# physiii/radio-mapper

Measured on AMD Instinct MI355X. Metric: IQ samples cross-correlated per second, higher is better.
Workload: dtype f32; 1 GPU; cfg3: 8 buoys (28 pairs), 10 MS/s complex64, N=4096-sample windows (L=8192), 4096 windows per GPU resident in HBM; n_buoys=8, n_pairs=28, n_samples=4096, windows_per_gpu=4096, channels=1, windows_total=4096, parallelism=windows sharded x1, no collective

## Files before the change

__graft_entry__.py:

```python
import os
import subprocess
import sys

ROOT = os.path.dirname(os.path.abspath(__file__))
CSRC = os.path.join(ROOT, "radio-mapper_amd", "csrc")
HIPCC = os.environ.get("HIPCC", "/opt/rocm/bin/hipcc")
HIP_FLAGS = ["--offload-arch=gfx950", "-O3", "-std=c++17", "-fPIC", "-shared", "-fno-slp-vectorize",
             "-mllvm", "-simplifycfg-sink-common=false",
             "-Wno-inline-asm"]
SOURCES = ("rmx_hip.hip", "fft_r16.hpp", "fft_r8.hpp", "kwin.hpp", "kwin8k.hpp", "kwin16k.hpp", "generic_path.hpp", "win_eo.hpp", "host_plan.hpp",
           "detect_path.hpp", "lag_bounds.hpp", "kwin_body.hpp", "xspec_weight.hpp", "integrate.hpp")
LIB = os.path.join(CSRC, "librmx_hip.so")
_MARK = b"RMX_BUILD_INFO source_digest="


def source_digest() -> str:
    import hashlib
    h = hashlib.sha256()
    for f in sorted(os.listdir(CSRC)):
        if f.endswith((".hip", ".hpp")):
            h.update(f.encode())
            h.update(open(os.path.join(CSRC, f), "rb").read())
    h.update(open(os.path.join(ROOT, "include", "rmx.h"), "rb").read())
    h.update(" ".join(HIP_FLAGS).encode())
    return h.hexdigest()[:16]


def binary_digest(path: str = LIB):
    try:
        blob = open(path, "rb").read()
    except OSError:
        return None
    k = blob.find(_MARK)
    if k < 0:
        return None
    k += len(_MARK)
    return blob[k:k + 16].decode("ascii", "replace")


def _stale(target=LIB) -> bool:
    return binary_digest(target) != source_digest()


def build(force: bool = False) -> None:
    for f in SOURCES:
        assert os.path.exists(os.path.join(CSRC, f)), f
    lib = LIB
    if force or _stale(lib):
        cmd = [HIPCC] + HIP_FLAGS + [f'-DRMX_SOURCE_DIGEST="{source_digest()}"', "-o", lib, os.path.join(CSRC, "rmx_hip.hip")]
        print("[build]", " ".join(cmd), flush=True)
        subprocess.run(cmd, check=True)
    else:
        print("[build] up to date (binary digest == source digest %s): no compile" % source_digest(), flush=True)
    if ROOT not in sys.path:
        sys.path.insert(0, ROOT)
    import radio_mapper_amd
    from radio_mapper_amd import xcorr
    lib_h = xcorr.load_library()
    assert lib_h.rmx_version() >= 1
    info = xcorr.build_info()
    assert info.get("source_digest") == source_digest(), (info, source_digest())
    print("[build] ok:", lib, info["text"], "devices visible:", xcorr.device_count(), flush=True)


def smoke() -> None:
    if ROOT not in sys.path:
        sys.path.insert(0, ROOT)
    import numpy as np
    import radio_mapper_amd as rm
    from radio_mapper_amd import xcorr
    from oracle import xcorr_ref as orc
    iq, delays, raw = rm.synth.make_windows(8, 4, 4096, 10e6, seed=7, return_u8=True)
    ri, rf, rp = orc.xcorr_batch_literal(iq)
    ref = ri + rf
    worst = 0.0
    for fused in (0, 1):
        with xcorr.XcorrEngine(4, 4096, 8, device=0) as eng:
            if fused:
                eng.set_option("small4096", 0)
            li, lf, pk = eng.correlate(iq)
            li8, lf8, pk8 = eng.correlate(raw)
        assert np.array_equal(li, ri), "integer lags differ from the oracle"
        assert np.all(np.abs(li + lf.astype(np.float64) - ref) <= 1e-5 * np.maximum(np.abs(ref), 1.0))
        assert np.allclose(pk, rp, rtol=1e-5)
        assert np.array_equal(li, li8) and np.array_equal(lf, lf8)
        worst = max(worst, float(np.abs(li + lf - ref).max()))
    print("[smoke] ok: 8 windows x 6 pairs through both N = 4096 paths, lag_int bit-exact, max |dlag| = %.2e" % worst, flush=True)


if __name__ == "__main__":
    build()
    if len(sys.argv) > 1 and sys.argv[1] == "smoke":
        smoke()
```

radio-mapper_amd/csrc/fft_r16.hpp:

```cpp
#pragma once
#include <hip/hip_runtime.h>

#include <type_traits>

namespace rmx {

constexpr int kM = 4096;
constexpr int kL = 2 * kM;
constexpr int kThreads = 512;
constexpr int kSlots = 16;

__device__ __forceinline__ float2 cmul(float2 a, float2 b) {
    return make_float2(a.x * b.x - a.y * b.y, a.x * b.y + a.y * b.x);
}
__device__ __forceinline__ float2 cadd(float2 a, float2 b) { return make_float2(a.x + b.x, a.y + b.y); }
__device__ __forceinline__ float2 csub(float2 a, float2 b) { return make_float2(a.x - b.x, a.y - b.y); }

__device__ __forceinline__ void dft4(float2& a0, float2& a1, float2& a2, float2& a3) {
    const float2 t0 = cadd(a0, a2), t1 = csub(a0, a2);
    const float2 t2 = cadd(a1, a3), t3 = csub(a1, a3);
    a0 = cadd(t0, t2);
    a2 = csub(t0, t2);
    a1 = make_float2(t1.x + t3.y, t1.y - t3.x);
    a3 = make_float2(t1.x - t3.y, t1.y + t3.x);
// ... 48 lines not shown
    const float ax = a.x, ay = a.y;
    a.x = b.x; a.y = b.y;
    b.x = ax; b.y = ay;
}

__device__ __forceinline__ void dft16_layer2(float2 (&v)[16]) {
    dft4(v[0], v[1], v[2], v[3]);
    dft4_tw<true>(v[4], v[5], v[6], v[7], make_float2(1.f, 0.f), make_float2(RMX_C1, -RMX_S1),
                  make_float2(RMX_RH, -RMX_RH), make_float2(RMX_S1, -RMX_C1));
    {
        float2 &a0 = v[8], &a1 = v[9], &a2 = v[10], &a3 = v[11];
        const float2 t0 = make_float2(a0.x + a2.y, a0.y - a2.x);
        const float2 t1 = make_float2(a0.x - a2.y, a0.y + a2.x);
        const float2 A1 = make_float2((a1.x + a1.y) * RMX_RH, (a1.y - a1.x) * RMX_RH);
        const float2 t2 = cfma(A1, a3, make_float2(-RMX_RH, -RMX_RH));
        const float2 t3 = twice_minus(A1, t2);
        dft4_tail(a0, a1, a2, a3, t0, t1, t2, t3);
    }
    dft4_tw<true>(v[12], v[13], v[14], v[15], make_float2(1.f, 0.f), make_float2(RMX_S1, -RMX_C1),
                  make_float2(-RMX_RH, -RMX_RH), make_float2(-RMX_C1, RMX_S1));
    swap2(v[1], v[4]);
    swap2(v[2], v[8]);
    swap2(v[3], v[12]);
    swap2(v[6], v[9]);
    swap2(v[7], v[13]);
    swap2(v[11], v[14]);
}

template <class F>
__device__ __forceinline__ void dft16_layer2_emit(float2 (&v)[16], F&& emit) {
    dft4(v[0], v[1], v[2], v[3]);
    emit(std::integral_constant<int, 0>{}, v[0], v[1], v[2], v[3]);
    __builtin_amdgcn_sched_barrier(0);
    dft4_tw<true>(v[4], v[5], v[6], v[7], make_float2(1.f, 0.f), make_float2(RMX_C1, -RMX_S1),
                  make_float2(RMX_RH, -RMX_RH), make_float2(RMX_S1, -RMX_C1));
    emit(std::integral_constant<int, 1>{}, v[4], v[5], v[6], v[7]);
    __builtin_amdgcn_sched_barrier(0);
    {
        float2 &a0 = v[8], &a1 = v[9], &a2 = v[10], &a3 = v[11];
        const float2 t0 = make_float2(a0.x + a2.y, a0.y - a2.x);
        const float2 t1 = make_float2(a0.x - a2.y, a0.y + a2.x);
        const float2 A1 = make_float2((a1.x + a1.y) * RMX_RH, (a1.y - a1.x) * RMX_RH);
        const float2 t2 = cfma(A1, a3, make_float2(-RMX_RH, -RMX_RH));
        const float2 t3 = twice_minus(A1, t2);
        dft4_tail(a0, a1, a2, a3, t0, t1, t2, t3);
    }
    emit(std::integral_constant<int, 2>{}, v[8], v[9], v[10], v[11]);
    __builtin_amdgcn_sched_barrier(0);
    dft4_tw<true>(v[12], v[13], v[14], v[15], make_float2(1.f, 0.f), make_float2(RMX_S1, -RMX_C1),
                  make_float2(-RMX_RH, -RMX_RH), make_float2(-RMX_C1, RMX_S1));
    emit(std::integral_constant<int, 3>{}, v[12], v[13], v[14], v[15]);
    __builtin_amdgcn_sched_barrier(0);
}

__device__ __forceinline__ void dft16(float2 (&v)[16]) {
    dft4(v[0], v[4], v[8], v[12]);
    dft4(v[1], v[5], v[9], v[13]);
    dft4(v[2], v[6], v[10], v[14]);
    dft4(v[3], v[7], v[11], v[15]);
    dft16_layer2(v);
}

template <bool W0_IS_ONE>
__device__ __forceinline__ void dft16_tw(float2 (&v)[16], const float2 (&w)[16]) {
    dft4_tw<W0_IS_ONE>(v[0], v[4], v[8], v[12], w[0], w[4], w[8], w[12]);
    dft4_tw<false>(v[1], v[5], v[9], v[13], w[1], w[5], w[9], w[13]);
    dft4_tw<false>(v[2], v[6], v[10], v[14], w[2], w[6], w[10], w[14]);
    dft4_tw<false>(v[3], v[7], v[11], v[15], w[3], w[7], w[11], w[15]);
    dft16_layer2(v);
}

struct C16 {
    float re[16], im[16];
    __device__ __forceinline__ float2 get(int q) const { return make_float2(re[q], im[q]); }
    __device__ __forceinline__ void set(int q, float x, float y) { re[q] = x; im[q] = y; }
};
template <bool W0_IS_ONE>
__device__ __forceinline__ void dft16_tw_l1(float2 (&v)[16], const C16& w) {
    dft4_tw<W0_IS_ONE>(v[0], v[4], v[8], v[12], w.get(0), w.get(4), w.get(8), w.get(12));
    dft4_tw<false>(v[1], v[5], v[9], v[13], w.get(1), w.get(5), w.get(9), w.get(13));
    dft4_tw<false>(v[2], v[6], v[10], v[14], w.get(2), w.get(6), w.get(10), w.get(14));
    dft4_tw<false>(v[3], v[7], v[11], v[15], w.get(3), w.get(7), w.get(11), w.get(15));
}
template <bool W0_IS_ONE>
__device__ __forceinline__ void dft16_tw(float2 (&v)[16], const C16& w) {
    dft16_tw_l1<W0_IS_ONE>(v, w);
    dft16_layer2(v);
}

__device__ __forceinline__ void dft16_tw_row_l1(float2 (&v)[16], const float4* row, float4 f0, float4 f1) {
    dft4_tw<true>(v[0], v[4], v[8], v[12], make_float2(1.0f, 0.0f), make_float2(f0.x, f0.y), make_float2(f0.z, f0.w),
                  make_float2(f1.x, f1.y));
    const float4 f2 = row[2], f3 = row[3];
    dft4_tw<false>(v[1], v[5], v[9], v[13], make_float2(f1.z, f1.w), make_float2(f2.x, f2.y), make_float2(f2.z, f2.w),
                   make_float2(f3.x, f3.y));
    const float4 f4 = row[4], f5 = row[5];
    dft4_tw<false>(v[2], v[6], v[10], v[14], make_float2(f3.z, f3.w), make_float2(f4.x, f4.y), make_float2(f4.z, f4.w),
                   make_float2(f5.x, f5.y));
    const float4 f6 = row[6], f7 = row[7];
    dft4_tw<false>(v[3], v[7], v[11], v[15], make_float2(f5.z, f5.w), make_float2(f6.x, f6.y), make_float2(f6.z, f6.w),
                   make_float2(f7.x, f7.y));
}
__device__ __forceinline__ void dft16_tw_row_l1(float2 (&v)[16], const float4* row) {
    dft16_tw_row_l1(v, row, row[0], row[1]);
}
__device__ __forceinline__ void dft16_tw_row(float2 (&v)[16], const float4* row, float4 f0, float4 f1) {
    dft16_tw_row_l1(v, row, f0, f1);
    dft16_layer2(v);
}
__device__ __forceinline__ void dft16_tw_row(float2 (&v)[16], const float4* row) {
    dft16_tw_row_l1(v, row);
    dft16_layer2(v);
}

__device__ __forceinline__ void cmul_inplace(float& x, float& y, float wr, float wi) {
    float tmp;
    asm volatile("v_mul_f32 %2, %0, %4\n\tv_mul_f32 %0, %0, %3\n\tv_fma_f32 %0, -%1, %4, %0\n\tv_fma_f32 %1, %1, %3, %2"
                 : "+v"(x), "+v"(y), "=&v"(tmp)
                 : "s"(wr), "s"(wi));
}

__device__ __forceinline__ void cmul4_inplace(float& x0, float& y0, float& x1, float& y1, float& x2, float& y2,
                                              float& x3, float& y3, float2 w0, float2 w1, float2 w2, float2 w3) {
    float tmp;
#define RMX_CM(X, Y, WR, WI)                                                                              \
    "v_mul_f32 %8, %" #X ", %" #WI "\n\tv_mul_f32 %" #X ", %" #X ", %" #WR "\n\tv_fma_f32 %" #X ", -%" #Y \
    ", %" #WI ", %" #X "\n\tv_fma_f32 %" #Y ", %" #Y ", %" #WR ", %8\n\t"
    asm volatile(RMX_CM(0, 1, 9, 10) RMX_CM(2, 3, 11, 12) RMX_CM(4, 5, 13, 14) RMX_CM(6, 7, 15, 16)
                 : "+v"(x0), "+v"(y0), "+v"(x1), "+v"(y1), "+v"(x2), "+v"(y2), "+v"(x3), "+v"(y3), "=&v"(tmp)
                 : "s"(w0.x), "s"(w0.y), "s"(w1.x), "s"(w1.y), "s"(w2.x), "s"(w2.y), "s"(w3.x), "s"(w3.y));
#undef RMX_CM
}

__device__ __forceinline__ float2 w32(int q) {
    constexpr float c[16] = {1.0f, 0.98078528040323044913f, 0.92387953251128675613f,
                             0.83146961230254523708f, 0.70710678118654752440f,
                             0.55557023301960222474f, 0.38268343236508977173f,
                             0.19509032201612826785f, 0.0f, -0.19509032201612826785f,
                             -0.38268343236508977173f, -0.55557023301960222474f,
                             -0.70710678118654752440f, -0.83146961230254523708f,
                             -0.92387953251128675613f, -0.98078528040323044913f};
    constexpr float s[16] = {0.0f, 0.19509032201612826785f, 0.38268343236508977173f,
                             0.55557023301960222474f, 0.70710678118654752440f,
                             0.83146961230254523708f, 0.92387953251128675613f,
                             0.98078528040323044913f, 1.0f, 0.98078528040323044913f,
                             0.92387953251128675613f, 0.83146961230254523708f,
                             0.70710678118654752440f, 0.55557023301960222474f,
                             0.38268343236508977173f, 0.19509032201612826785f};
    return make_float2(c[q], -s[q]);
}

constexpr int kBcRow = 34;
constexpr int kBcHalf = 16 * kBcRow;
constexpr int kXchgF2 = 16 * kBcHalf;

__device__ __forceinline__ void wave_lds_fence() {
    __builtin_amdgcn_fence(__ATOMIC_RELEASE, "wavefront");
    __builtin_amdgcn_s_waitcnt(0xC07F);
    __builtin_amdgcn_wave_barrier();
    __builtin_amdgcn_fence(__ATOMIC_ACQUIRE, "wavefront");
}

__device__ __forceinline__ void wave_lds_order() {
    __builtin_amdgcn_fence(__ATOMIC_RELEASE, "wavefront");
    __builtin_amdgcn_wave_barrier();
    __builtin_amdgcn_fence(__ATOMIC_ACQUIRE, "wavefront");
// ... 184 lines not shown
```

radio-mapper_amd/csrc/kwin.hpp:

```cpp
#pragma once
#include <hip/hip_runtime.h>

#include <cmath>
#include <type_traits>
#include <vector>

#include "fft_r16.hpp"

#ifndef RMX_KWIN_LOAD_AUX
#define RMX_KWIN_LOAD_AUX 0
#endif
#ifndef RMX_KWIN_STORE_AUX
#define RMX_KWIN_STORE_AUX 0
#endif

namespace rmx {

using u32x4 = unsigned int __attribute__((ext_vector_type(4)));
using u32x2 = unsigned int __attribute__((ext_vector_type(2)));
using f32x4 = float __attribute__((ext_vector_type(4)));
using f32x2 = float __attribute__((ext_vector_type(2)));

constexpr int kLdsXchg = kXchgF2 * 8;
constexpr int kLdsTw2 = 16 * kTw2RowF2 * 8;
constexpr int kLdsRed = 64;
constexpr int kLdsBytes = kLdsXchg + kLdsTw2 + kLdsRed;

__device__ __forceinline__ void load_tw2_to_lds(float2* tw2_lds, const float2* __restrict__ tw2_g, int t) {
    if (t < 256) tw2_lds[(t >> 4) * kTw2RowF2 + (t & 15)] = tw2_g[t];
}

__device__ __forceinline__ void load_tw2_to_lds_grouped(float2* tw2_lds, const float2* __restrict__ tw2_g, int t) {
    if (t < 256) {
        const int a = t >> 4, q = t & 15;
        tw2_lds[a * kTw2RowF2 + (q == 0 ? 15 : 4 * (q & 3) + (q >> 2) - 1)] = tw2_g[t];
    }
}

__device__ __forceinline__ void load_tw1(float2 (&tw1)[16], const float4* __restrict__ tw1_g, int t) {
#pragma unroll
    for (int j = 0; j < 8; ++j) {
        const float4 w = tw1_g[j * kThreads + t];
        tw1[2 * j] = make_float2(w.x, w.y);
        tw1[2 * j + 1] = make_float2(w.z, w.w);
    }
}

constexpr int kLdsWinImg = kLdsXchg;
constexpr int kLdsWinTw2 = 2 * kLdsWinImg;
#ifdef RMX_KWIN_PEAK2
constexpr int kResSlots = 4;
constexpr int kResBatch = 3;
constexpr int kHaloRows = 7;
#ifndef RMX_KWIN_RES_MASK
#define RMX_KWIN_RES_MASK 3
#endif
#else
#ifndef RMX_KWIN_RES_MASK
#define RMX_KWIN_RES_MASK 7
#endif
constexpr int kResSlots = 8;
constexpr int kResBatch = 7;
constexpr int kHaloRows = 4;
#endif
constexpr int kLdsWinHalo = kLdsWinTw2 + kLdsTw2;
constexpr int kLdsWinRed = kLdsWinHalo + kResSlots * 8 * kHaloRows * 16 * 4;
constexpr int kLdsWinOidx = kLdsWinRed + kResSlots * 8 * 16;
constexpr int kLdsWinBytes = kLdsWinOidx + kResSlots * 4;
static_assert(kLdsWinBytes <= 160 * 1024, "k_win LDS");

__device__ __forceinline__ void k_to_owner(int kk, int& tt, int& q) {
    const int par = (kk >= kM - 1) ? 0 : 1;
    const int n = par ? (kk + 1) : (kk - (kM - 1));
    tt = 2 * (n & 255) + par;
    q = n >> 8;
}

template <bool BOUNDED = false>
__device__ __forceinline__ void resolve_batch(int lane, const float4* red, const float* halo, const int* oidx,
                                              int first, int cnt, long obase, float out_scale,
                                              int* __restrict__ lag_int, float* __restrict__ lag_frac,
                                              float* __restrict__ peak, LagBounds lb = {}, long w = 0) {
    const int g = lane >> 3, r = lane & 7;
    const bool act = g < cnt;
    const int slot = (first + g) & (kResSlots - 1);
    const float* rf = reinterpret_cast<const float*>(red) + 4 * (slot * 8 + r);
    const int* ri = reinterpret_cast<const int*>(rf);
    const float ex = act ? rf[0] : -3.0f;
    const int k = act ? ri[1] : 0x7fffffff;
    const float tm = rf[2], tp = rf[3];
    const int out = oidx[slot];
    float gmax = ex;
    gmax = fmaxf(gmax, __builtin_bit_cast(float, dpp_i<0xB1>(__builtin_bit_cast(int, gmax))));
    gmax = fmaxf(gmax, __builtin_bit_cast(float, dpp_i<0x4E>(__builtin_bit_cast(int, gmax))));
    gmax = fmaxf(gmax, __builtin_bit_cast(float, dpp_i<0x141>(__builtin_bit_cast(int, gmax))));
    int kstar = (ex == gmax) ? k : 0x7fffffff;
// ... 160 lines not shown
```

radio-mapper_amd/csrc/kwin_body.hpp:

```cpp
#ifdef RMX_ABLATE
    const int dbg = dbg_rt;
#else
    constexpr int dbg = 0;
    (void)dbg_rt;
#endif
    extern __shared__ __attribute__((aligned(16))) char smem[];
    float2* img0 = reinterpret_cast<float2*>(smem);
    float2* img1 = reinterpret_cast<float2*>(smem + kLdsWinImg);
    float2* tw2_lds = reinterpret_cast<float2*>(smem + kLdsWinTw2);
    float* halo = reinterpret_cast<float*>(smem + kLdsWinHalo);
    float4* red = reinterpret_cast<float4*>(smem + kLdsWinRed);
    int* oidx = reinterpret_cast<int*>(smem + kLdsWinOidx);

    const int t = threadIdx.x;
    const int p = t & 1, u = t >> 1;
    const int lane = t & 63, wave = t >> 6;
    const int B = n_buoys;
    const int n_pairs = B * (B - 1) / 2;

    load_tw2_to_lds_grouped(tw2_lds, tw2_g, t);
    float2 tw1[16];
    load_tw1(tw1, tw1_g, t);
#ifndef RMX_KWIN_LDS1
    const float4* tw2row = reinterpret_cast<const float4*>(tw2_lds + (t & 15) * kTw2RowF2);
// ... 73 lines not shown
                resolve_batch(lane, red, halo, oidx, (npair - npend) & (kResSlots - 1), npend, obase, out_scale, lag_int,
                              lag_frac, peak);
            }
#endif
            npend = 0;
        }
    };
    auto mul_w32_odd = [&](float2 (&v)[16]) __attribute__((always_inline)) {
        if (p) {
            {
#pragma unroll
                for (int q = 1; q < 4; ++q) {
                    const float2 w = w32(q);
                    float x = v[q].x, y = v[q].y;
                    cmul_inplace(x, y, w.x, w.y);
                    v[q].x = x;
                    v[q].y = y;
                }
            }
#pragma unroll
            for (int q = 4; q < 16; q += 4) {
                float x0 = v[q].x, y0 = v[q].y, x1 = v[q + 1].x, y1 = v[q + 1].y;
                float x2 = v[q + 2].x, y2 = v[q + 2].y, x3 = v[q + 3].x, y3 = v[q + 3].y;
                cmul4_inplace(x0, y0, x1, y1, x2, y2, x3, y3, w32(q), w32(q + 1), w32(q + 2), w32(q + 3));
                v[q].x = x0; v[q].y = y0; v[q + 1].x = x1; v[q + 1].y = y1;
                v[q + 2].x = x2; v[q + 2].y = y2; v[q + 3].x = x3; v[q + 3].y = y3;
            }
        }
    };
    const int samp_bytes = U8 ? 2 : 8;
    const __amdgpu_buffer_rsrc_t xs = __builtin_amdgcn_make_buffer_rsrc(
        const_cast<char*>(reinterpret_cast<const char*>(iq_v)) + (first_window + wl) * (long)B * kM * samp_bytes, 0,
        B * kM * samp_bytes, 0x00020000);
    const __amdgpu_buffer_rsrc_t ss = __builtin_amdgcn_make_buffer_rsrc(
        reinterpret_cast<char*>(spec) + wbase * (long)(8 * kThreads * 16), 0, B * (8 * kThreads * 16), 0x00020000);
    const int xoff = u * samp_bytes, soff = t * 16;
    auto load_x = [&](C16& d, int b) __attribute__((always_inline)) {
        if constexpr (U8) {
#pragma unroll
            for (int q = 0; q < 16; ++q)
                d.re[q] = __uint_as_float((unsigned)__builtin_amdgcn_raw_buffer_load_b16(xs, xoff, (b * kM + q * 256) * 2, 0));
        } else {
#pragma unroll
            for (int q = 0; q < 16; ++q) {
                const u32x2 r = __builtin_amdgcn_raw_buffer_load_b64(xs, xoff, (b * kM + q * 256) * 8, 0);
                d.set(q, __uint_as_float(r.x), __uint_as_float(r.y));
            }
        }
    };
    auto load_x_part_from = [&](const __amdgpu_buffer_rsrc_t& rs, C16& d, int b, auto part) __attribute__((always_inline)) {
        constexpr int G = decltype(part)::value;
        if (dbg & 64) return;
#ifndef RMX_KWIN_NO_SPREAD
        constexpr int Q0 = 2 * G, Q1 = 2 * G + 2;
#else
        constexpr int Q0 = 4 * G, Q1 = 4 * G + 4;
#endif
        int bo = b * (kM * samp_bytes);
        asm volatile("" : "+s"(bo));
        if constexpr (U8) {
#pragma unroll
            for (int q = Q0; q < Q1; ++q)
                d.re[q] = __uint_as_float((unsigned)__builtin_amdgcn_raw_buffer_load_b16(rs, xoff, bo + q * 256 * 2, 0));
        } else {
#pragma unroll
            for (int q = Q0; q < Q1; ++q) {
                const u32x2 r = __builtin_amdgcn_raw_buffer_load_b64(rs, xoff, bo + q * 256 * 8, 0);
                d.set(q, __uint_as_float(r.x), __uint_as_float(r.y));
            }
        }
    };
    auto load_x_part = [&](C16& d, int b, auto part) __attribute__((always_inline)) { load_x_part_from(xs, d, b, part); };
    auto cvt_x = [&](C16& d) __attribute__((always_inline)) {
        if constexpr (U8) {
#pragma unroll
            for (int q = 0; q < 16; ++q) {
                const unsigned r = __float_as_uint(d.re[q]);
                d.set(q, (float)(r & 0xffu) - 127.5f, (float)(r >> 8) - 127.5f);
            }
        }
    };
    auto load_spec_part = [&](C16& d, int b, auto part) __attribute__((always_inline)) {
        constexpr int G = decltype(part)::value;
        if (dbg & 32) b = 1;
        if (dbg & 128) return;
#ifndef RMX_KWIN_NO_SPREAD
        constexpr int J0 = G, J1 = G + 1;
#else
        constexpr int J0 = 2 * G, J1 = 2 * G + 2;
#endif
        int bo = b * (8 * kThreads * 16);
        asm volatile("" : "+s"(bo));
#pragma unroll
        for (int j = J0; j < J1; ++j) {
            const u32x4 w = __builtin_amdgcn_raw_buffer_load_b128(ss, soff, bo + j * (kThreads * 16), RMX_KWIN_LOAD_AUX);
            d.set(2 * j, __uint_as_float(w.x), __uint_as_float(w.y));
            d.set(2 * j + 1, __uint_as_float(w.z), __uint_as_float(w.w));
        }
    };
    auto store_spec = [&](const C16& d, int b) __attribute__((always_inline)) {
#pragma unroll
        for (int j = 0; j < 8; ++j) {
            float e0 = d.re[2 * j], e1 = d.im[2 * j], e2 = d.re[2 * j + 1], e3 = d.im[2 * j + 1];
            asm volatile("" : "+v"(e0), "+v"(e1), "+v"(e2), "+v"(e3));
            const u32x4 w = {__float_as_uint(e0), __float_as_uint(e1), __float_as_uint(e2), __float_as_uint(e3)};
            __builtin_amdgcn_raw_buffer_store_b128(w, ss, soff + (b * 8 + j) * (kThreads * 16), 0, RMX_KWIN_STORE_AUX);
        }
    };
    auto fwd = [&](C16& xc) __attribute__((always_inline)) {
        float2* img = (seq & 1) ? img1 : img0;
        float2 x[16];
#ifdef RMX_KWIN_STAMPS
        RMX_LAP(6);
        asm volatile("s_waitcnt vmcnt(0)" ::: "memory");
        RMX_LAP(7);
#endif
#pragma unroll
        for (int q = 0; q < 16; ++q) x[q] = xc.get(q);
        mul_w32_odd(x);
        dft16(x);
        mul_tw1(x, tw1);
#ifndef RMX_KWIN_LDS1
        if (!(dbg & 8)) xchg_a2_write(img, x, t);
        RMX_LAP(0);
        barrier_hook(false);
        RMX_LAP(1);
        if (!(dbg & 8)) xchg_b2_read(img, x, t);
#else
        if (!(dbg & 8)) xchg_a_write(img, x, t);
        barrier_hook(false);
        if (!(dbg & 8)) xchg_b_read(img, x, t);
#endif
        dft16(x);
#ifdef RMX_TW2_LDS
        const float4 r0 = tw2row[0], r1 = tw2row[1];
#endif
        if (!(dbg & 4)) {
#ifndef RMX_KWIN_LDS1
        loc_write16(loc_m0[seq & 1], x);
        wave_lds_order();
        loc_read16(smem + (seq & 1) * kLdsWinImg + loc_rd, x);
#else
        xchg_bc_write_b(img, x, t);
        wave_lds_order();
        xchg_bc_read_c(img, x, t);
#endif
        }
#ifndef RMX_TW2_LDS
        dft16_tw<true>(x, tw2r);
#else
        dft16_tw_row(x, tw2row, r0, r1);
#endif
#pragma unroll
        for (int q = 0; q < 16; ++q) xc.set(q, x[q].x, x[q].y);
        ++seq;
        RMX_LAP(2);
    };
    auto pair_h1 = [&](const C16& a, const C16& s, int tr, auto prefetch) __attribute__((always_inline)) {
        float2* img = (tr & 1) ? img1 : img0;
        float2 v[16];
#ifdef RMX_KWIN_STAMPS
        {
            const long long c0 = __builtin_readcyclecounter();
            asm volatile("s_waitcnt vmcnt(0)" ::: "memory");
            const long long c1 = __builtin_readcyclecounter();
            stamp_vm += (int)(c1 - c0);
        }
#endif
#pragma unroll
        for (int q = 0; q < 16; ++q) v[q] = make_float2(s.im[q], s.re[q]);
        dft16_tw_l1<false>(v, a);
#pragma unroll
        for (int q = 0; q < 16; q += 4)
            asm volatile("" : "+v"(v[q].x), "+v"(v[q].y), "+v"(v[q + 1].x), "+v"(v[q + 1].y), "+v"(v[q + 2].x),
                         "+v"(v[q + 2].y), "+v"(v[q + 3].x), "+v"(v[q + 3].y));
        __builtin_amdgcn_sched_barrier(0);
        {
            float2* wb = img + (u >> 4) * kBcHalf + (u & 15) * kBcRow + p;
            (void)wb;
            dft16_layer2_emit(v, [&](auto kac, const float2& x0, const float2& x1, const float2& x2, const float2& x3)
                                     __attribute__((always_inline)) {
                constexpr int ka = decltype(kac)::value;
                if (!(dbg & 4)) {
#ifndef RMX_KWIN_LDS1
                    loc_write4<ka, ka + 4, ka + 8, ka + 12>(loc_m0[tr & 1], x0, x1, x2, x3);
#else
                    wb[2 * ka] = make_float2(x0.x, x0.y);
                    wb[2 * (ka + 4)] = make_float2(x1.x, x1.y);
                    wb[2 * (ka + 8)] = make_float2(x2.x, x2.y);
                    wb[2 * (ka + 12)] = make_float2(x3.x, x3.y);
#endif
                }
                if (!(dbg & 16)) prefetch(kac);
            });
        }
#ifdef RMX_TW2_LDS
        const float4 r0 = tw2row[0], r1 = tw2row[1];
#endif
        if (!(dbg & 4)) {
            wave_lds_order();
#ifndef RMX_KWIN_LDS1
            loc_read16(smem + (tr & 1) * kLdsWinImg + loc_rd, v);
#else
            xchg_bc_read_b(img, v, t);
#endif
        }
#ifndef RMX_TW2_LDS
        dft16_tw_l1<true>(v, tw2r);
#else
        dft16_tw_row_l1(v, tw2row, r0, r1);
#endif
        {
#ifndef RMX_KWIN_LDS1
            float2* xb = img + xb2_base(t);
#else
            float2* xb = img + (u >> 4) * kBcHalf + (u & 15) * 2 + p;
#endif
            dft16_layer2_emit(v, [&](auto kac, const float2& x0, const float2& x1, const float2& x2, const float2& x3)
                                     __attribute__((always_inline)) {
                constexpr int ka = decltype(kac)::value;
                if (!(dbg & 8)) {
                    xb[ka * 32] = make_float2(x0.x, x0.y);
                    xb[(ka + 4) * 32] = make_float2(x1.x, x1.y);
                    xb[(ka + 8) * 32] = make_float2(x2.x, x2.y);
                    xb[(ka + 12) * 32] = make_float2(x3.x, x3.y);
                }
#ifndef RMX_KWIN_NO_SPREAD
                if (!(dbg & 16)) prefetch(std::integral_constant<int, ka + 4>{});
#endif
            });
        }
    };
    auto pair_h2 = [&](int tr, int out_idx) __attribute__((always_inline)) {
        const float2* img = (tr & 1) ? img1 : img0;
        const int rb = npair & (kResSlots - 1);
        float2 v[16];
#ifndef RMX_KWIN_LDS1
        if (!(dbg & 8)) xchg_a2_read(img, v, t);
#else
        if (!(dbg & 8)) xchg_a_read(img, v, t);
#endif
        dft16_tw<false>(v, tw1);
        mul_w32_odd(v);
        pair_fmac8(v[0].x, v[0].y, v[1].x, v[1].y, v[2].x, v[2].y, v[3].x, v[3].y, sgn);
        pair_fmac8(v[4].x, v[4].y, v[5].x, v[5].y, v[6].x, v[6].y, v[7].x, v[7].y, sgn);
        pair_fmac8(v[8].x, v[8].y, v[9].x, v[9].y, v[10].x, v[10].y, v[11].x, v[11].y, sgn);
        pair_fmac8(v[12].x, v[12].y, v[13].x, v[13].y, v[14].x, v[14].y, v[15].x, v[15].y, sgn);
        float mag[16];
#pragma unroll
        for (int q = 0; q < 16; ++q) mag[q] = fmaf(v[q].x, v[q].x, v[q].y * v[q].y);
        if (p && u == 0) mag[0] = -1.0f;
        if constexpr (BOUNDED) {
            int klo, khi;
            lag_window(lb, first_window + wl, out_idx, kM - 1, klo, khi);
// ... 90 lines not shown
#pragma unroll
            for (int q4 = 0; q4 < 4; ++q4)
                hp[q4] = make_float4(mag[4 * q4], mag[4 * q4 + 1], mag[4 * q4 + 2], mag[4 * q4 + 3]);
        }
        float tmax = mag[0];
#pragma unroll
        for (int q = 1; q < 16; ++q) tmax = fmaxf(tmax, mag[q]);
#ifndef RMX_KWIN_OLD_PEAK
        int qa = 16, qb = 16, qc = 16, qd = 16;
        float wrow;
        {
            unsigned long long k0, k1, k2, k3;
#define RMX_AS4(M0, M1, M2, M3, Q)                                                        \
    "v_cmp_eq_f32_e64 %[k0], %[" #M0 "], %[t]\n\tv_cmp_eq_f32_e64 %[k1], %[" #M1 "], %[t]\n\t" \
    "v_cmp_eq_f32_e64 %[k2], %[" #M2 "], %[t]\n\tv_cmp_eq_f32_e64 %[k3], %[" #M3 "], %[t]\n\t" \
    "v_cndmask_b32_e64 %[qa], %[qa], " #Q ", %[k0]\n\tv_cndmask_b32_e64 %[qb], %[qb], " #Q "+1, %[k1]\n\t" \
    "v_cndmask_b32_e64 %[qc], %[qc], " #Q "+2, %[k2]\n\tv_cndmask_b32_e64 %[qd], %[qd], " #Q "+3, %[k3]\n\t"
            asm volatile(RMX_AS4(mc, md, me, mf, 12)
                         "v_max_f32_dpp %[w], %[t], %[t] quad_perm:[1,0,3,2] row_mask:0xf bank_mask:0xf\n\t"
                         RMX_AS4(m8, m9, ma, mb, 8)
                         "v_max_f32_dpp %[w], %[w], %[w] quad_perm:[2,3,0,1] row_mask:0xf bank_mask:0xf\n\t"
                         RMX_AS4(m4, m5, m6, m7, 4)
                         "v_max_f32_dpp %[w], %[w], %[w] row_half_mirror row_mask:0xf bank_mask:0xf\n\t"
                         RMX_AS4(m0, m1, m2, m3, 0)
                         "v_max_f32_dpp %[w], %[w], %[w] row_mirror row_mask:0xf bank_mask:0xf"
                         : [qa] "+v"(qa), [qb] "+v"(qb), [qc] "+v"(qc), [qd] "+v"(qd), [w] "=&v"(wrow), [k0] "=&s"(k0),
                           [k1] "=&s"(k1), [k2] "=&s"(k2), [k3] "=&s"(k3)
                         : [t] "v"(tmax), [m0] "v"(mag[0]), [m1] "v"(mag[1]), [m2] "v"(mag[2]), [m3] "v"(mag[3]),
                           [m4] "v"(mag[4]), [m5] "v"(mag[5]), [m6] "v"(mag[6]), [m7] "v"(mag[7]), [m8] "v"(mag[8]),
                           [m9] "v"(mag[9]), [ma] "v"(mag[10]), [mb] "v"(mag[11]), [mc] "v"(mag[12]), [md] "v"(mag[13]),
                           [me] "v"(mag[14]), [mf] "v"(mag[15]));
#undef RMX_AS4
        }
        const int qsel = min(min(qa, qb), min(qc, qd));
        const int kq = kbase + qsel * 256;
        const int wi = __builtin_bit_cast(int, wrow);
        const float wmax = fmaxf(fmaxf(__builtin_bit_cast(float, __builtin_amdgcn_readlane(wi, 0)),
                                       __builtin_bit_cast(float, __builtin_amdgcn_readlane(wi, 16))),
                                 fmaxf(__builtin_bit_cast(float, __builtin_amdgcn_readlane(wi, 32)),
                                       __builtin_bit_cast(float, __builtin_amdgcn_readlane(wi, 48))));
        const unsigned long long hit = __ballot(tmax == wmax);
        int kw, ls, qs;
        if (__popcll(hit) == 1) {
            ls = __ffsll((long long)hit) - 1;
            kw = __builtin_amdgcn_readlane(kq, ls);
            qs = __builtin_amdgcn_readlane(qsel, ls);
        } else {
            kw = wave_min_i32(tmax == wmax ? kq : 0x7fffffff);
            int ts;
            k_to_owner(kw, ts, qs);
            ls = ts & 63;
        }
#else
        int qa = 16, qb = 16, qc = 16, qd = 16;
        argsel4<12>(qa, qb, qc, qd, mag[12], mag[13], mag[14], mag[15], tmax);
        argsel4<8>(qa, qb, qc, qd, mag[8], mag[9], mag[10], mag[11], tmax);
        argsel4<4>(qa, qb, qc, qd, mag[4], mag[5], mag[6], mag[7], tmax);
        argsel4<0>(qa, qb, qc, qd, mag[0], mag[1], mag[2], mag[3], tmax);
        const int qsel = min(min(qa, qb), min(qc, qd));
        const int kq = kbase + qsel * 256;
        const float wmax = wave_max_f32(tmax);
        const int kw = wave_min_i32(tmax == wmax ? kq : 0x7fffffff);
        int ts, qs;
        k_to_owner(kw, ts, qs);
        const int ls = ts & 63;
#endif
        typedef float f16v __attribute__((ext_vector_type(16)));
        const f16v mv = {mag[0], mag[1], mag[2],  mag[3],  mag[4],  mag[5],  mag[6],  mag[7],
                         mag[8], mag[9], mag[10], mag[11], mag[12], mag[13], mag[14], mag[15]};
        const float sel = mv[__builtin_amdgcn_readfirstlane(qs)];
        const int seli = __builtin_bit_cast(int, sel);
        const float tapm = ls >= 2 ? __builtin_bit_cast(float, __builtin_amdgcn_readlane(seli, ls >= 2 ? ls - 2 : 0)) : -2.0f;
        const float tapp = ls <= 61 ? __builtin_bit_cast(float, __builtin_amdgcn_readlane(seli, ls <= 61 ? ls + 2 : 63)) : -2.0f;
        if (lane == 0) {
            const u32x4 rec = {__float_as_uint(wmax), (unsigned)kw, __float_as_uint(tapm), __float_as_uint(tapp)};
            *reinterpret_cast<u32x4*>(red + rb * 8 + wave) = rec;
            if (wave == 0) oidx[rb] = out_idx;
        }
#endif
        ++npend;
        ++npair;
    };
    auto pair = [&](const C16& a, const C16& s, int out_idx, auto prefetch) __attribute__((always_inline)) {
        pair_h1(a, s, seq, prefetch);
        RMX_LAP(4);
        barrier_hook(false);
        RMX_LAP(5);
        pair_h2(seq, out_idx);
        RMX_LAP(6);
        ++seq;
    };
    auto out_of = [&](int i, int j) -> int { return i * B - (i * (i + 1)) / 2 + (j - i - 1); };

    RMX_STAMP(0);
    load_x(sa, 0);
    if (B > 1) load_x(sb, 1);
    cvt_x(sa);
    fwd(sa);
    for (int e = 1; e + 1 < B; ++e) {
        cvt_x(sb);
        fwd(sb);
        store_spec(sb, e);
        RMX_LAP(3);
        pair(sa, sb, out_of(0, e), [&](auto part) __attribute__((always_inline)) { load_x_part(sb, e + 1, part); });
    }
    if (B > 1) {
        cvt_x(sb);
        fwd(sb);
        store_spec(sb, B - 1);
        RMX_LAP(3);
        pair(sa, sb, out_of(0, B - 1), [&](auto part) __attribute__((always_inline)) {
            if (B > 2) {
                load_spec_part(sa, 1, part);
                load_spec_part(sb, B - 1, part);
            }
        });
    }
    RMX_STAMP(1);
#ifdef RMX_KWIN_STAMPS
    lap_on = false;
#endif
    {
        const int M2 = (B - 1) * (B - 2) / 2;
        const bool late_h2 = stag == 1 ? ((wave >> 1) & 1) : stag == 2 ? (wave & 1) : stag == 3 ? (wave >> 2) :
                             stag == 4 ? ((wave ^ (wave >> 2)) & 1) : (stag == 5);
        auto j_of = [&](int i, int s) -> int { return (i & 1) ? (B - 1 - s) : (i + 1 + s); };
        int ci = 1, cs = 0;
        int ni = 1, ns = 1;
        if (ns >= B - 1 - ni) { ++ni; ns = 0; }
        auto h1_of = [&](int hi, int hs, int tr) __attribute__((always_inline)) {
            int pi = hi, ps = hs + 1;
            if (ps >= B - 1 - pi) { ++pi; ps = 0; }
            const bool valid = pi + 1 < B;
#ifdef RMX_KWIN_FORCE_ANCHOR
            const bool new_anchor = valid;
#else
            const bool new_anchor = valid && pi != hi;
#endif
#ifndef RMX_KWIN_REQ_BRANCHY
            const int pj = valid ? j_of(pi, ps) : B - 1;
            pair_h1(sa, sb, tr, [&](auto part) __attribute__((always_inline)) {
                if constexpr (decltype(part)::value == 0) {
                    if (new_anchor) {
                        load_spec_part(sa, pi, std::integral_constant<int, 0>{});
                        load_spec_part(sa, pi, std::integral_constant<int, 1>{});
                        load_spec_part(sa, pi, std::integral_constant<int, 2>{});
                        load_spec_part(sa, pi, std::integral_constant<int, 3>{});
                        load_spec_part(sa, pi, std::integral_constant<int, 4>{});
                        load_spec_part(sa, pi, std::integral_constant<int, 5>{});
                        load_spec_part(sa, pi, std::integral_constant<int, 6>{});
                        load_spec_part(sa, pi, std::integral_constant<int, 7>{});
                    }
                }
                load_spec_part(sb, pj, part);
            });
#else
            const int pj = j_of(pi, ps);
            pair_h1(sa, sb, tr, [&](auto part) __attribute__((always_inline)) {
                if (valid) {
                    if (pi != hi) load_spec_part(sa, pi, part);
                    load_spec_part(sb, pj, part);
                }
            });
#endif
        };
        if (M2 > 0) h1_of(ci, cs, seq);
        for (int m = 0; m < M2; ++m) {
            barrier_hook(false);
            const bool has_next = m + 1 < M2;
            const int out_idx = out_of(ci, j_of(ci, cs));
#ifndef RMX_KWIN_PRIO_MODE
#define RMX_KWIN_PRIO_MODE 1
#endif
#if !defined(RMX_KWIN_PRIO) && !defined(RMX_KWIN_NO_PRIO)
#define RMX_KWIN_PRIO 1
#endif
#ifdef RMX_KWIN_PRIO
#if RMX_KWIN_PRIO_MODE == 2
            if (wave >= 4) { if (late_h2) __builtin_amdgcn_s_setprio(0); else __builtin_amdgcn_s_setprio(RMX_KWIN_PRIO); }
#define RMX_PRIO_MID() do { if (wave >= 4) { if (late_h2) __builtin_amdgcn_s_setprio(RMX_KWIN_PRIO); else __builtin_amdgcn_s_setprio(0); } } while (0)
#else
            if (wave >= 4) __builtin_amdgcn_s_setprio(RMX_KWIN_PRIO);
#define RMX_PRIO_MID() do { if (wave >= 4) __builtin_amdgcn_s_setprio(0); } while (0)
#endif
#else
#define RMX_PRIO_MID() do { } while (0)
#endif
#ifdef RMX_KWIN_STAMPS
            const long long p0 = __builtin_readcyclecounter();
            long long p1;
#define RMX_PIECE_MID() p1 = __builtin_readcyclecounter()
#else
#define RMX_PIECE_MID() do { } while (0)
#endif
            if (late_h2) {
                if (has_next) h1_of(ni, ns, seq + 1);
                RMX_PRIO_MID();
                RMX_PIECE_MID();
                pair_h2(seq, out_idx);
            } else {
                pair_h2(seq, out_idx);
                RMX_PRIO_MID();
                RMX_PIECE_MID();
                if (has_next) h1_of(ni, ns, seq + 1);
            }
#ifdef RMX_KWIN_STAMPS
            {
                const long long p2 = __builtin_readcyclecounter();
                stamp_pc1 += (int)(p1 - p0);
                stamp_pc2 += (int)(p2 - p1);
            }
#endif
#undef RMX_PIECE_MID
#undef RMX_PRIO_MID
            ++seq;
            ci = ni; cs = ns;
            ++ns;
            if (ns >= B - 1 - ni) { ++ni; ns = 0; }
        }
    }
    RMX_STAMP(2);
#ifdef RMX_KWIN_STAMPS
    if (lane == 0 && (wl / (int)gridDim.x) < 64) {
        rmx_stamps_vm[((int)blockIdx.x * 64 + wl / (int)gridDim.x) * 8 + wave] = stamp_vm;
        rmx_stamps_bar[(((int)blockIdx.x * 64 + wl / (int)gridDim.x) * 8 + wave) * 2] = stamp_drain;
        rmx_stamps_bar[(((int)blockIdx.x * 64 + wl / (int)gridDim.x) * 8 + wave) * 2 + 1] = stamp_bar;
        for (int k = 0; k < 8; ++k) rmx_stamps_p1[(((int)blockIdx.x * 64 + wl / (int)gridDim.x) * 8 + wave) * 8 + k] = lap_acc[k];
        rmx_stamps_pc[(((int)blockIdx.x * 64 + wl / (int)gridDim.x) * 8 + wave) * 2] = stamp_pc1;
        rmx_stamps_pc[(((int)blockIdx.x * 64 + wl / (int)gridDim.x) * 8 + wave) * 2 + 1] = stamp_pc2;
    }
#endif
    seq = 0;
    barrier_hook(true);
    }
```

Measured before the change: 276.4 billion samples/s.

## Reorder pair schedule so next anchor spectrum is handed over in registers

Introduces a pair-scheduling header that reorders phase-1 and phase-2 buoy visitation so the last stream spectrum of each run becomes the next anchor. The anchor is then copied register-to-register instead of reloaded from global memory, which removes the full 8-part anchor reload at each anchor change. It also skips storing one spectrum, specializes the last h1 step so it issues no prefetch, and changes the FMA ordering of the first twiddle layer. The risks are extra register moves, a changed output index mapping, and slightly different rounding.

Result: no change. 279.0 billion samples/s (median of 6 runs) (+0.9%).

```diff
diff --git a/__graft_entry__.py b/__graft_entry__.py
--- a/__graft_entry__.py
+++ b/__graft_entry__.py
@@ -9,7 +9,7 @@
              "-mllvm", "-simplifycfg-sink-common=false",
              "-Wno-inline-asm"]
 SOURCES = ("rmx_hip.hip", "fft_r16.hpp", "fft_r8.hpp", "kwin.hpp", "kwin8k.hpp", "kwin16k.hpp", "generic_path.hpp", "win_eo.hpp", "host_plan.hpp",
-           "detect_path.hpp", "lag_bounds.hpp", "kwin_body.hpp", "xspec_weight.hpp", "integrate.hpp")
+           "detect_path.hpp", "lag_bounds.hpp", "kwin_body.hpp", "kwin_sched.hpp", "xspec_weight.hpp", "integrate.hpp")
 LIB = os.path.join(CSRC, "librmx_hip.so")
 _MARK = b"RMX_BUILD_INFO source_digest="
 
diff --git a/radio-mapper_amd/csrc/fft_r16.hpp b/radio-mapper_amd/csrc/fft_r16.hpp
--- a/radio-mapper_amd/csrc/fft_r16.hpp
+++ b/radio-mapper_amd/csrc/fft_r16.hpp
@@ -154,6 +154,29 @@
     dft4_tw<false>(v[2], v[6], v[10], v[14], w.get(2), w.get(6), w.get(10), w.get(14));
     dft4_tw<false>(v[3], v[7], v[11], v[15], w.get(3), w.get(7), w.get(11), w.get(15));
 }
+template <bool XFIRST>
+__device__ __forceinline__ float2 cmul_ord(float2 a, float2 b) {
+    if constexpr (XFIRST) return make_float2(fmaf(-a.y, b.y, a.x * b.x), fmaf(a.y, b.x, a.x * b.y));
+    else return make_float2(fmaf(a.x, b.x, -(a.y * b.y)), fmaf(a.x, b.y, a.y * b.x));
+}
+template <bool XFIRST>
+__device__ __forceinline__ void dft4_tw_ord(float2& a0, float2& a1, float2& a2, float2& a3, float2 w0, float2 w1,
+                                            float2 w2, float2 w3) {
+    const float2 A0 = cmul_ord<XFIRST>(a0, w0);
+    const float2 t0 = cfma(A0, a2, w2);
+    const float2 t1 = twice_minus(A0, t0);
+    const float2 A1 = cmul_ord<XFIRST>(a1, w1);
+    const float2 t2 = cfma(A1, a3, w3);
+    const float2 t3 = twice_minus(A1, t2);
+    dft4_tail(a0, a1, a2, a3, t0, t1, t2, t3);
+}
+template <bool XFIRST>
+__device__ __forceinline__ void dft16_tw_l1_ord(float2 (&v)[16], const C16& w) {
+    dft4_tw_ord<XFIRST>(v[0], v[4], v[8], v[12], w.get(0), w.get(4), w.get(8), w.get(12));
+    dft4_tw_ord<XFIRST>(v[1], v[5], v[9], v[13], w.get(1), w.get(5), w.get(9), w.get(13));
+    dft4_tw_ord<XFIRST>(v[2], v[6], v[10], v[14], w.get(2), w.get(6), w.get(10), w.get(14));
+    dft4_tw_ord<XFIRST>(v[3], v[7], v[11], v[15], w.get(3), w.get(7), w.get(11), w.get(15));
+}
 template <bool W0_IS_ONE>
 __device__ __forceinline__ void dft16_tw(float2 (&v)[16], const C16& w) {
     dft16_tw_l1<W0_IS_ONE>(v, w);
diff --git a/radio-mapper_amd/csrc/kwin.hpp b/radio-mapper_amd/csrc/kwin.hpp
--- a/radio-mapper_amd/csrc/kwin.hpp
+++ b/radio-mapper_amd/csrc/kwin.hpp
@@ -6,12 +6,16 @@
 #include <vector>
 
 #include "fft_r16.hpp"
+#include "kwin_sched.hpp"
 
 #ifndef RMX_KWIN_LOAD_AUX
 #define RMX_KWIN_LOAD_AUX 0
 #endif
 #ifndef RMX_KWIN_STORE_AUX
 #define RMX_KWIN_STORE_AUX 0
+#endif
+#ifndef RMX_KWIN_LAST_H1
+#define RMX_KWIN_LAST_H1 1
 #endif
 
 namespace rmx {
diff --git a/radio-mapper_amd/csrc/kwin_body.hpp b/radio-mapper_amd/csrc/kwin_body.hpp
--- a/radio-mapper_amd/csrc/kwin_body.hpp
+++ b/radio-mapper_amd/csrc/kwin_body.hpp
@@ -179,7 +179,7 @@
     };
     auto load_spec_part = [&](C16& d, int b, auto part) __attribute__((always_inline)) {
         constexpr int G = decltype(part)::value;
-        if (dbg & 32) b = 1;
+        if (dbg & 32) b = 2;
         if (dbg & 128) return;
 #ifndef RMX_KWIN_NO_SPREAD
         constexpr int J0 = G, J1 = G + 1;
@@ -253,7 +253,7 @@
         ++seq;
         RMX_LAP(2);
     };
-    auto pair_h1 = [&](const C16& a, const C16& s, int tr, auto prefetch) __attribute__((always_inline)) {
+    auto pair_h1 = [&](const C16& a, const C16& s, int tr, auto xfirst, auto prefetch) __attribute__((always_inline)) {
         float2* img = (tr & 1) ? img1 : img0;
         float2 v[16];
 #ifdef RMX_KWIN_STAMPS
@@ -266,7 +266,7 @@
 #endif
 #pragma unroll
         for (int q = 0; q < 16; ++q) v[q] = make_float2(s.im[q], s.re[q]);
-        dft16_tw_l1<false>(v, a);
+        dft16_tw_l1_ord<decltype(xfirst)::value>(v, a);
 #pragma unroll
         for (int q = 0; q < 16; q += 4)
             asm volatile("" : "+v"(v[q].x), "+v"(v[q].y), "+v"(v[q + 1].x), "+v"(v[q + 1].y), "+v"(v[q + 2].x),
@@ -523,7 +523,7 @@
         ++npair;
     };
     auto pair = [&](const C16& a, const C16& s, int out_idx, auto prefetch) __attribute__((always_inline)) {
-        pair_h1(a, s, seq, prefetch);
+        pair_h1(a, s, seq, std::false_type{}, prefetch);
         RMX_LAP(4);
         barrier_hook(false);
         RMX_LAP(5);
@@ -531,30 +531,34 @@
         RMX_LAP(6);
         ++seq;
     };
-    auto out_of = [&](int i, int j) -> int { return i * B - (i * (i + 1)) / 2 + (j - i - 1); };
+    namespace ks = kwin_sched;
+    auto out_of = [&](int i, int j) -> int { return ks::out_of(B, i, j); };
+    auto hand_over = [&]() __attribute__((always_inline)) {
+        asm volatile("");
+#pragma unroll
+        for (int q = 0; q < 16; ++q) sa.set(q, sb.re[q], sb.im[q]);
+    };
 
     RMX_STAMP(0);
     load_x(sa, 0);
-    if (B > 1) load_x(sb, 1);
+    if (B > 1) load_x(sb, ks::phase1_buoy(B, 1));
     cvt_x(sa);
     fwd(sa);
-    for (int e = 1; e + 1 < B; ++e) {
+    for (int k = 1; k + 1 < B; ++k) {
+        const int e = ks::phase1_buoy(B, k), nx = ks::phase1_buoy(B, k + 1);
         cvt_x(sb);
         fwd(sb);
         store_spec(sb, e);
         RMX_LAP(3);
-        pair(sa, sb, out_of(0, e), [&](auto part) __attribute__((always_inline)) { load_x_part(sb, e + 1, part); });
+        pair(sa, sb, out_of(0, e), [&](auto part) __attribute__((always_inline)) { load_x_part(sb, nx, part); });
     }
     if (B > 1) {
         cvt_x(sb);
         fwd(sb);
-        store_spec(sb, B - 1);
         RMX_LAP(3);
-        pair(sa, sb, out_of(0, B - 1), [&](auto part) __attribute__((always_inline)) {
-            if (B > 2) {
-                load_spec_part(sa, 1, part);
-                load_spec_part(sb, B - 1, part);
-            }
+        pair(sa, sb, out_of(0, 1), [&](auto part) __attribute__((always_inline)) {
+            if constexpr (decltype(part)::value == 0) hand_over();
+            if (B > 2) load_spec_part(sb, B - 1, part);
         });
     }
     RMX_STAMP(1);
@@ -565,47 +569,39 @@
         const int M2 = (B - 1) * (B - 2) / 2;
         const bool late_h2 = stag == 1 ? ((wave >> 1) & 1) : stag == 2 ? (wave & 1) : stag == 3 ? (wave >> 2) :
                              stag == 4 ? ((wave ^ (wave >> 2)) & 1) : (stag == 5);
-        auto j_of = [&](int i, int s) -> int { return (i & 1) ? (B - 1 - s) : (i + 1 + s); };
+        auto j_of = [&](int i, int s) -> int { return __builtin_amdgcn_readfirstlane(ks::stream_of(B, i, s)); };
         int ci = 1, cs = 0;
-        int ni = 1, ns = 1;
-        if (ns >= B - 1 - ni) { ++ni; ns = 0; }
-        auto h1_of = [&](int hi, int hs, int tr) __attribute__((always_inline)) {
-            int pi = hi, ps = hs + 1;
-            if (ps >= B - 1 - pi) { ++pi; ps = 0; }
-            const bool valid = pi + 1 < B;
-#ifdef RMX_KWIN_FORCE_ANCHOR
-            const bool new_anchor = valid;
-#else
-            const bool new_anchor = valid && pi != hi;
-#endif
-#ifndef RMX_KWIN_REQ_BRANCHY
-            const int pj = valid ? j_of(pi, ps) : B - 1;
-            pair_h1(sa, sb, tr, [&](auto part) __attribute__((always_inline)) {
-                if constexpr (decltype(part)::value == 0) {
-                    if (new_anchor) {
-                        load_spec_part(sa, pi, std::integral_constant<int, 0>{});
-                        load_spec_part(sa, pi, std::integral_constant<int, 1>{});
-                        load_spec_part(sa, pi, std::integral_constant<int, 2>{});
-                        load_spec_part(sa, pi, std::integral_constant<int, 3>{});
-                        load_spec_part(sa, pi, std::integral_constant<int, 4>{});
-                        load_spec_part(sa, pi, std::integral_constant<int, 5>{});
-                        load_spec_part(sa, pi, std::integral_constant<int, 6>{});
-                        load_spec_part(sa, pi, std::integral_constant<int, 7>{});
-                    }
+        int ni = ks::next(B, ks::Pos{ci, cs}).i, ns = ks::next(B, ks::Pos{ci, cs}).s;
+        auto h1_of = [&](int hi, int hs, int tr, auto last) __attribute__((always_inline)) {
+            const ks::Pos nx = ks::next(B, ks::Pos{hi, hs});
+            const int pi = nx.i, ps = nx.s;
+            if constexpr (std::is_same_v<decltype(last), std::true_type>) {
+                pair_h1(sa, sb, tr, std::true_type{}, [&](auto) __attribute__((always_inline)) {});
+            } else {
+                const bool hand = pi != hi;
+                if constexpr (std::is_same_v<decltype(last), std::false_type>) {
+                    const int pj = j_of(pi, ps);
+                    pair_h1(sa, sb, tr, std::true_type{}, [&](auto part) __attribute__((always_inline)) {
+                        if constexpr (decltype(part)::value == 0) {
+                            if (hand) hand_over();
+                        }
+                        load_spec_part(sb, pj, part);
+                    });
+                } else {
+                    const bool req = !last;
+                    const int pj = req ? j_of(pi, ps) : 2;
+                    pair_h1(sa, sb, tr, std::true_type{}, [&](auto part) __attribute__((always_inline)) {
+                        if (req) {
+                            if constexpr (decltype(part)::value == 0) {
+                                if (hand) hand_over();
+                            }
+                            load_spec_part(sb, pj, part);
+                        }
+                    });
                 }
-                load_spec_part(sb, pj, part);
-            });
-#else
-            const int pj = j_of(pi, ps);
-            pair_h1(sa, sb, tr, [&](auto part) __attribute__((always_inline)) {
-                if (valid) {
-                    if (pi != hi) load_spec_part(sa, pi, part);
-                    load_spec_part(sb, pj, part);
-                }
-            });
-#endif
+            }
         };
-        if (M2 > 0) h1_of(ci, cs, seq);
+        if (M2 > 0) h1_of(ci, cs, seq, (int)(M2 == 1));
         for (int m = 0; m < M2; ++m) {
             barrier_hook(false);
             const bool has_next = m + 1 < M2;
@@ -634,8 +630,13 @@
 #else
 #define RMX_PIECE_MID() do { } while (0)
 #endif
+#if RMX_KWIN_LAST_H1 == 1
+#define RMX_NEXT_H1() do { if (m + 2 < M2) h1_of(ni, ns, seq + 1, std::false_type{}); else if (has_next) h1_of(ni, ns, seq + 1, std::true_type{}); } while (0)
+#else
+#define RMX_NEXT_H1() do { if (has_next) h1_of(ni, ns, seq + 1, (int)(m + 2 >= M2)); } while (0)
+#endif
             if (late_h2) {
-                if (has_next) h1_of(ni, ns, seq + 1);
+                RMX_NEXT_H1();
                 RMX_PRIO_MID();
                 RMX_PIECE_MID();
                 pair_h2(seq, out_idx);
@@ -643,8 +644,9 @@
                 pair_h2(seq, out_idx);
                 RMX_PRIO_MID();
                 RMX_PIECE_MID();
-                if (has_next) h1_of(ni, ns, seq + 1);
-            }
+                RMX_NEXT_H1();
+            }
+#undef RMX_NEXT_H1
 #ifdef RMX_KWIN_STAMPS
             {
                 const long long p2 = __builtin_readcyclecounter();
@@ -656,8 +658,7 @@
 #undef RMX_PRIO_MID
             ++seq;
             ci = ni; cs = ns;
-            ++ns;
-            if (ns >= B - 1 - ni) { ++ni; ns = 0; }
+            { const ks::Pos nn = ks::next(B, ks::Pos{ni, ns}); ni = nn.i; ns = nn.s; }
         }
     }
     RMX_STAMP(2);
diff --git a/radio-mapper_amd/csrc/kwin_sched.hpp b/radio-mapper_amd/csrc/kwin_sched.hpp
--- /dev/null
+++ b/radio-mapper_amd/csrc/kwin_sched.hpp
@@ -0,0 +1,51 @@
+#pragma once
+
+#ifndef RMX_KWIN_ORDER
+#define RMX_KWIN_ORDER 0
+#endif
+
+namespace rmx {
+namespace kwin_sched {
+
+constexpr int kOrder = RMX_KWIN_ORDER;
+
+constexpr int out_of(int B, int i, int j) { return i * B - (i * (i + 1)) / 2 + (j - i - 1); }
+
+constexpr int phase1_buoy(int B, int k) { return k == 0 ? 0 : (k + 1 < B ? k + 1 : 1); }
+constexpr bool phase1_stores(int e) { return e >= 2; }
+constexpr bool seam_handover(int B) { return B > 2; }
+constexpr int seam_request(int B) { return B > 2 ? B - 1 : -1; }
+
+constexpr int phase2_pairs(int B) { return B > 2 ? (B - 1) * (B - 2) / 2 : 0; }
+constexpr int run_len(int B, int i) { return B - 1 - i; }
+constexpr int stream_of(int B, int i, int s) {
+    return ((i & 1) || kOrder == 1) ? B - 1 - s : (s + 1 < run_len(B, i) ? i + 2 + s : i + 1);
+}
+
+struct Pos {
+    int i, s;
+};
+constexpr Pos first_pos() { return Pos{1, 0}; }
+constexpr Pos next(int B, Pos p) { return p.s + 1 < run_len(B, p.i) ? Pos{p.i, p.s + 1} : Pos{p.i + 1, 0}; }
+constexpr bool valid(int B, Pos p) { return p.i + 1 < B; }
+
+struct Pair {
+    int anchor, stream;
+    int out;
+    bool handover;
+    int request;
+};
+constexpr Pair pair_at(int B, Pos p) {
+    const Pos n = next(B, p);
+    const bool more = valid(B, n);
+    const int j = stream_of(B, p.i, p.s);
+    return Pair{p.i, j, out_of(B, p.i, j), more && n.i != p.i, more ? stream_of(B, n.i, n.s) : -1};
+}
+constexpr Pair pair_of(int B, int m) {
+    Pos p = first_pos();
+    for (int k = 0; k < m; ++k) p = next(B, p);
+    return pair_at(B, p);
+}
+
+}
+}
```
